# seqan/lambda

Measured on AMD Instinct MI355X. Metric: GCUPS (gapped extension, full-rectangle parity mode; pass-1 cells per second of whole step) searchp BLOSUM62, higher is better.
Workload: dtype f16x2 (exact small integers) + int32

## Files before the change

lambda_amd/csrc/lx_ckpt.hip:

```cpp
#include <hip/hip_runtime.h>

#include <algorithm>
#include <cstdio>
#include <cstdlib>

#include "lx_aids.h"
#include "lx_dp_common.h"

namespace lx
{

#ifndef LX_CKPT_EVERY
#define LX_CKPT_EVERY 16
#endif
constexpr int kCkptEvery = LX_CKPT_EVERY;
#ifndef LX_CKPT_UNROLL
#define LX_CKPT_UNROLL 4
#endif
#define LX_CKPT_PRAGMA(x) _Pragma(#x)
#define LX_CKPT_UNROLL_N(n) LX_CKPT_PRAGMA(unroll n)
#define LX_CKPT_UNROLL_PRAGMA LX_CKPT_UNROLL_N(LX_CKPT_UNROLL)
#ifndef LX_BT_TILE_AT
#define LX_BT_TILE_AT 40
#endif
#ifndef LX_BT_WAVES
#define LX_BT_WAVES 2
#endif
#ifndef LX_BT_HOPS
#define LX_BT_HOPS 2
#endif
#ifndef LX_BT_REFILL_AT
#define LX_BT_REFILL_AT 24
#endif
#ifndef LX_BT_POOL
#define LX_BT_POOL 32
#endif
#ifndef LX_CKPT_FWD_WAVES
#define LX_CKPT_FWD_WAVES 4
#endif
#ifdef LX_BT_COUNT
__device__ unsigned long long lx_bt_counts[5];
#endif

template <int G>
__host__ __device__ constexpr uint32_t bnd_quad_index(uint32_t quad, uint32_t g)
{
    return quad * G + g;
}
#ifndef LX_CKPT_ROWCK_LANE_MAJOR
#define LX_CKPT_ROWCK_LANE_MAJOR 1
#endif
template <int G, int kCkDw>
__host__ __device__ constexpr uint32_t rowck_quad_index(uint32_t m, uint32_t g, uint32_t x)
{
    return LX_CKPT_ROWCK_LANE_MAJOR ? (m * G + g) * (kCkDw / 4) + x : (m * (kCkDw / 4) + x) * G + g;
}
template <int G, int C>
struct CkptLayout
{
    static constexpr int kCkDw = (C + 3) / 4 * 4;
    __host__ __device__ static constexpr uint64_t bnd_dwords(uint32_t steps_cap) { return (uint64_t)steps_cap * G; }
    __host__ __device__ static constexpr uint64_t slot_dwords(uint32_t steps_cap)
    {
        return bnd_dwords(steps_cap) + (uint64_t)(steps_cap / kCkptEvery) * G * kCkDw;
    }
};

__device__ __forceinline__ uint32_t pack16(int lo, int hi)
{
    return ((uint32_t)lo & 0xffffu) | ((uint32_t)hi << 16);
}

template <int G, int C, bool KNOWN, bool MULTI>
__global__ __launch_bounds__(64, (KNOWN ? LX_CKPT_FWD_WAVES : 3)) void ckpt_forward_kernel(TraceParams p)
{
    using Geo = ScoreGeo<G, C>;
    using Lay = CkptLayout<G, C>;
    extern __shared__ uint32_t lds[];

    int const  lane     = threadIdx.x;
    int const  grp      = lane / G;
    int const  g        = lane % G;
    bool const is_first = (g == 0);
    bool const is_last  = (g == G - 1);

    uint64_t const e     = (uint64_t)blockIdx.x * Geo::kGroups + grp;
    uint64_t       limit = p.n;
    if (p.count_ptr)
    {
        uint64_t const total = *p.count_ptr;
        limit = total > p.chunk_start ? min(p.n, total - p.chunk_start) : 0;
        if ((uint64_t)blockIdx.x * Geo::kGroups >= limit)
            return;
    }
    bool active = e < limit;
    if (active && p.src && p.src[e] == 0xffffffffu)
        active = false;
    bool in_list = e < limit;
    if constexpr (!KNOWN)
    {
        if (p.fixup)
        {
            bool const mine = in_list && p.score_out[e] == -1;
            if (__ballot(mine) == 0)
                return;
            active  = active && mine;
            in_list = mine;
        }
    }

    ScoringDev const * __restrict__ sc = p.sc;
    int const      ge    = sc->ge;
    int const      g2    = sc->g2;
    int const      nrows = p.nrows;
    uint32_t const padt  = (uint32_t)(nrows - 1);

    int             lq = 0, ls = 0;
    uint8_t const * q = p.q_res;
    uint8_t const * s = p.s_res;
    uint64_t        q_off = 0;
    if (e < limit)
    {
        Extension const x = p.ext[e];
        lq    = (int)x.q_len;
// ... 289 lines not shown
            grow   = take ? orow : grow;
            gtie   = take ? ot : gtie;
        }
        bool const take = gbest > run_best;
        run_best  = take ? gbest : run_best;
        run_strip = take ? (MULTI ? panel * G : 0) + gstrip : run_strip;
        run_row   = take ? grow : run_row;
        run_tie   = take ? gtie : run_tie;
    }
    if constexpr (MULTI)
    {
        if (npanels > 1)
        {
            __builtin_amdgcn_fence(__ATOMIC_RELEASE, "workgroup");
            __builtin_amdgcn_s_waitcnt(0);
            __builtin_amdgcn_fence(__ATOMIC_ACQUIRE, "workgroup");
        }
    }
    __builtin_amdgcn_wave_barrier();
    }

    if constexpr (KNOWN)
    {
#pragma unroll
        for (int off = 1; off < G; off <<= 1)
        {
            int const  oc = __shfl_xor(kcol, off), orow = __shfl_xor(krow, off);
            bool const take = oc < kcol;
            kcol = take ? oc : kcol;
            krow = take ? orow : krow;
        }
        if (in_list && is_first)
        {
            EndCell ec{};
            if (bad || (tgt > 0 && kcol == 0x7fffffff))
                ec.score = -1;
            else if (tgt > 0)
            {
                ec.score = tgt;
                ec.q_end = kcol + 1;
                ec.s_end = krow + 1;
            }
            p.ends[e] = ec;
        }
    }
    else
    {
        int const gbest = run_best, gstrip = run_strip, grow = run_row, gtie = run_tie;
        if (in_list && is_first)
        {
            EndCell ec{};
            if (bad)
                ec.score = -1;
            else if (active && gbest > 0)
            {
                ec.score = gbest;
                ec.q_end = -(gstrip + 1);
                ec.s_end = grow + 1;
                ec.flags = (gtie ? kEndAmbiguous : 0) | (int32_t)(ovf_tag << kEndOverflowShift);
            }
            p.ends[e] = ec;
            if (p.score_out)
                p.score_out[e] = bad ? -1 : (active ? gbest : 0);
        }
    }
}

template <int G, int C>
__global__ __launch_bounds__(64, LX_BT_WAVES) void ckpt_backtrace_kernel(TraceParams p)
{
    using Lay               = CkptLayout<G, C>;
    using L16               = Ckpt16Layout<G, C>;
    constexpr int kNibDw    = (C + 7) / 8;
    constexpr int kFar      = -(1 << 28);
    static_assert(kCkptEvery == 16, "the diagonal shortcut reads at most 16 residues per sequence");
    __shared__ int8_t   smat4[kAlph * kAlph];
    __shared__ int8_t   smat1n[kAlph * kAlph];
    __shared__ uint32_t tiles[kCkptEvery * kNibDw * 64];
    constexpr int kRecQ  = 10;
    constexpr int kLdsWg = 20 * 1024 - (int)sizeof(uint32_t) * kCkptEvery * kNibDw * 64 - 2 * kAlph * kAlph;
    constexpr int kPool  = LX_BT_POOL < kLdsWg / (16 * kRecQ) ? LX_BT_POOL : kLdsWg / (16 * kRecQ);
    static_assert(kPool >= 0 && kPool <= 64, "pool masks are 64 bits wide");
    __shared__ uint4 pool[kRecQ][kPool > 0 ? kPool : 1];
    for (int x = threadIdx.x; x < kAlph * kAlph; x += blockDim.x)
    {
        int const v = p.sc->mat[x];
        smat4[x]    = (int8_t)((v < -32 || v > 31) ? -125 : 4 * v + 3);
        smat1n[x]   = (int8_t)(x == kAlph * kAlph - 1 ? 0 : min(-v, 127));
    }
    __syncthreads();
    uint32_t const lane  = threadIdx.x;
    uint64_t       limit = p.n;
    if (p.count_ptr)
    {
        uint64_t const total = *p.count_ptr;
        limit = total > p.chunk_start ? min(p.n, total - p.chunk_start) : 0;
    }
    int const ge = p.sc->ge, g2 = p.sc->g2;
    int const ge4 = 4 * p.sc->ge, go4 = 4 * p.sc->go;
    uint64_t panel_dw = Lay::slot_dwords(p.steps_cap), panel16_dw = L16::slot_dwords(p.steps_cap), bnd_dw = Lay::bnd_dwords(p.steps_cap);

    bool             have = false, blocked = false, done = false, need_col = false, scan = false, c16 = false;
    uint64_t         po = 0;
    uint64_t         pos = 0;
    EndCell          ec{};
    uint32_t const * slot = nullptr;
    uint32_t         oct_mul = G, ck_mul = G * (L16::kCkDw / 4);
    uint64_t         ck16_off = 0;
    uint8_t const *  q = nullptr, * s = nullptr;
    uint8_t *        ops_al = nullptr;
    uint32_t         cap = 0, a0 = 0, apos = 0, acc = 0, n = 0;
    int              lq = 0, ls = 0;
    int              i = 0, j = 0, end_i = 0, end_j = 0;
    int              res_col = C, res_row = 0x7fffffff;
    int              nar_cw = C, nar_j0 = 0x7fffffff, nar_st0 = 0x7fffffff;
    auto locate = [&](int aj, int & st, int & j0, int & cw)
    {
        if (aj >= nar_j0)
        {
            int const jl = aj - nar_j0;
            int const gl = nar_cw == (3 * C + 3) / 4 ? jl / ((3 * C + 3) / 4) : nar_cw == (C + 1) / 2 ? jl / ((C + 1) / 2) : jl / ((C + 3) / 4);
            st = nar_st0 + gl;
            j0 = nar_j0 + gl * nar_cw;
            cw = nar_cw;
        }
        else
        {
            st = aj / C;
            j0 = st * C;
            cw = C;
        }
    };
    int              mode = 0;
    int              left = 0;
    int32_t          nm = 0, nx = 0, np = 0, go = 0, gx = 0;
    bool const       rle_mode = p.rle != nullptr;
    uint32_t         run_op = 3, run_len = 0, ncodes = 0;

    auto dec = [](uint32_t bits16) -> int { return (int)(int16_t)bits16; };
    auto expand = [](uint32_t code16) -> uint32_t
    {
        uint32_t const H = code16 & 0x7ffu;
        return H | ((H - (code16 >> 11)) << 16);
    };
    auto bnd_of = [&](uint32_t pn) { return reinterpret_cast<uint4 const *>(slot + (uint64_t)pn * (c16 ? panel16_dw : panel_dw)); };
    auto rowck_of = [&](uint32_t pn)
    {
        return reinterpret_cast<uint4 const *>(slot + (c16 ? (uint64_t)pn * panel16_dw + ck16_off
                                                           : (uint64_t)pn * panel_dw + bnd_dw));
    };
    auto oct16_index = [&](uint32_t o, uint32_t g_) -> uint32_t { return o * oct_mul + g_; };
    auto ck16_index  = [&](uint32_t m_, uint32_t g_, uint32_t x_) -> uint32_t { return m_ * ck_mul + g_ * (L16::kCkDw / 4) + x_; };
    auto rowck_word = [&](uint32_t m, uint32_t st, uint32_t c) -> uint32_t
    {
        if (c16)
            return expand(reinterpret_cast<uint16_t const *>(rowck_of(st / G) + ck16_index(m, st % G, c / 8))[c % 8]);
        return reinterpret_cast<uint32_t const *>(rowck_of(st / G) + rowck_quad_index<G, Lay::kCkDw>(m, st % G, c / 4))[c % 4];
    };
    auto bnd_word_of = [&](uint32_t st, uint32_t k) -> uint32_t
    {
        if (c16)
            return expand(reinterpret_cast<uint16_t const *>(bnd_of(st / G) + oct16_index(k / 8, st % G))[k & 7]);
        return reinterpret_cast<uint32_t const *>(bnd_of(st / G) + bnd_quad_index<G>(k / 4, st % G))[k & 3];
    };
    auto put_byte = [&](uint32_t byte)
    {
        acc |= byte << (8 * (apos & 3));
        if ((apos & 3) == 0)
        {
            if (apos + 3 <= a0 + cap - 1)
                *reinterpret_cast<uint32_t *>(ops_al + apos) = acc;
            else
                for (uint32_t b = 0; b < 4 && apos + b <= a0 + cap - 1; ++b)
                    ops_al[apos + b] = (uint8_t)(acc >> (8 * b));
            acc = 0;
        }
        --apos;
    };
    auto emit = [&](uint32_t op)
    {
        if (rle_mode)
        {
            uint32_t const oc = op == (uint32_t)'M' ? 0u : (op == (uint32_t)'D' ? 1u : 2u);
            if (oc != run_op || run_len == 64)
            {
                if (run_op != 3)
                {
                    put_byte((run_op << 6) | (run_len - 1));
                    ++ncodes;
                }
                run_op  = oc;
                run_len = 0;
            }
            ++run_len;
        }
        else
            put_byte(op);
        ++n;
    };

    auto begin_extension = [&](uint64_t e)
    {
        uint64_t oi = e;
        if (p.src)
        {
            uint32_t const sidx = p.src[e];
            if (sidx == 0xffffffffu)
                return;
            oi = sidx;
        }
        pos                = e;
        po                 = p.out_by_pos ? e : oi;
        uint64_t const  se = p.slot_by_src ? oi : e;
        ec                 = p.ends[se];
        Extension const x  = p.ext[e];
        if (ec.score <= 0)
        {
            Hsp out{};
            out.score     = ec.score < 0 ? -1 : 0;
            p.out_hsp[po] = out;
            return;
        }
        c16                = (ec.flags & kEndCompact) != 0;
        uint32_t const ovf = (uint32_t)ec.flags >> kEndOverflowShift;
        slot               = ovf ? p.ovf + (uint64_t)(ovf - 1) * p.ovf_stride : p.trace + se * p.slot_stride;
        uint32_t steps_e   = p.steps_cap;
        if (p.wf_tab && !ovf)
        {
            WfSlots const  t      = p.wf_tab[se / 16];
            uint64_t const stride = (uint64_t)t.panels_cap * (c16 ? L16::slot_dwords(t.steps_cap) : Lay::slot_dwords(t.steps_cap));
            slot                  = ((p.split_n != 0 && se >= p.split_n) ? p.trace2 : p.trace) + t.off_dw + (se % 16) * stride;
            steps_e               = t.steps_cap;
        }
        panel_dw           = Lay::slot_dwords(steps_e);
        panel16_dw         = L16::slot_dwords(steps_e);
        bnd_dw             = Lay::bnd_dwords(steps_e);
        oct_mul            = G;
        ck_mul             = G * (L16::kCkDw / 4);
        ck16_off           = L16::bnd_dwords(steps_e);
        if (!ovf && (ec.flags & kEndWaveSlots))
        {
            constexpr uint32_t kW = 128 / G;
            uint64_t const     w  = se % kW;
            slot     = p.trace + (se - w) * p.slot_stride + w * (G * 4);
            oct_mul  = kW * G;
            ck_mul   = kW * G * (L16::kCkDw / 4);
// ... 87 lines not shown
            out.s_begin            = i + 1;
            out.s_end              = end_i + 1;
            out.n_ops              = (int32_t)n;
            out.num_matches        = nm;
            out.num_mismatches     = nx;
            out.num_positives      = np;
            out.num_gap_opens      = go;
            out.num_gap_extensions = gx;
            out.ops_shift          = rle_mode ? (int32_t)(uint32_t)at : (int32_t)(cap - n);
        }
        p.out_hsp[po] = out;
        if (rle_mode && p.rle_len)
            p.rle_len[pos] = ec.score > 0 ? ncodes : 0u;
        have          = false;
    };

    auto park = [&](uint32_t e)
    {
        uint32_t const flags = (blocked ? 1u : 0u) | (done ? 2u : 0u) | (need_col ? 4u : 0u) | (scan ? 8u : 0u) | (c16 ? 16u : 0u) |
                               ((uint32_t)mode << 5) | (run_op << 7) | (run_len << 9) | (a0 << 16) | ((uint32_t)nar_cw << 18) |
                               ((uint32_t)res_col << 24);
        uint64_t const sp = reinterpret_cast<uintptr_t>(slot), qp = reinterpret_cast<uintptr_t>(q), spp = reinterpret_cast<uintptr_t>(s),
                       op = reinterpret_cast<uintptr_t>(ops_al);
        pool[0][e] = make_uint4(flags, (uint32_t)pos, (uint32_t)po, (uint32_t)ec.score);
        pool[1][e] = make_uint4((uint32_t)sp, (uint32_t)(sp >> 32), oct_mul, ck_mul);
        pool[2][e] = make_uint4((uint32_t)ck16_off, (uint32_t)panel_dw, (uint32_t)panel16_dw, (uint32_t)bnd_dw);
        pool[3][e] = make_uint4((uint32_t)qp, (uint32_t)(qp >> 32), (uint32_t)spp, (uint32_t)(spp >> 32));
        pool[4][e] = make_uint4((uint32_t)op, (uint32_t)(op >> 32), cap, apos);
        pool[5][e] = make_uint4(acc, n, (uint32_t)lq, (uint32_t)ls);
        pool[6][e] = make_uint4((uint32_t)i, (uint32_t)j, (uint32_t)end_i, (uint32_t)end_j);
        pool[7][e] = make_uint4((uint32_t)res_row, (uint32_t)nar_j0, (uint32_t)nar_st0, (uint32_t)left);
        pool[8][e] = make_uint4((uint32_t)nm, (uint32_t)nx, (uint32_t)np, (uint32_t)go);
        pool[9][e] = make_uint4((uint32_t)gx, ncodes, 0u, 0u);
    };
    auto unpark = [&](uint4 const (&r)[kRecQ])
    {
        uint32_t const flags = r[0].x;
        blocked  = (flags & 1u) != 0;
        done     = (flags & 2u) != 0;
        need_col = (flags & 4u) != 0;
        scan     = (flags & 8u) != 0;
        c16      = (flags & 16u) != 0;
        mode     = (int)((flags >> 5) & 3u);
        run_op   = (flags >> 7) & 3u;
        run_len  = (flags >> 9) & 127u;
        a0       = (flags >> 16) & 3u;
        nar_cw   = (int)((flags >> 18) & 63u);
        res_col  = (int)((flags >> 24) & 63u);
        pos      = r[0].y;
        po       = r[0].z;
        ec.score = (int32_t)r[0].w;
        slot     = reinterpret_cast<uint32_t const *>(((uint64_t)r[1].y << 32) | r[1].x);
        oct_mul  = r[1].z;
        ck_mul   = r[1].w;
        ck16_off   = r[2].x;
        panel_dw   = r[2].y;
        panel16_dw = r[2].z;
        bnd_dw     = r[2].w;
        q      = reinterpret_cast<uint8_t const *>(((uint64_t)r[3].y << 32) | r[3].x);
        s      = reinterpret_cast<uint8_t const *>(((uint64_t)r[3].w << 32) | r[3].z);
        ops_al = reinterpret_cast<uint8_t *>(((uint64_t)r[4].y << 32) | r[4].x);
        cap    = r[4].z;
        apos   = r[4].w;
        acc    = r[5].x;
        n      = r[5].y;
        lq     = (int)r[5].z;
        ls     = (int)r[5].w;
        i      = (int)r[6].x;
        j      = (int)r[6].y;
        end_i  = (int)r[6].z;
        end_j  = (int)r[6].w;
        res_row = (int)r[7].x;
        nar_j0  = (int)r[7].y;
        nar_st0 = (int)r[7].z;
        left    = (int)r[7].w;
        nm      = (int32_t)r[8].x;
        nx      = (int32_t)r[8].y;
        np      = (int32_t)r[8].z;
        go      = (int32_t)r[8].w;
        gx      = (int32_t)r[9].x;
        ncodes  = r[9].y;
        have    = true;
    };
    auto nth_bit = [](uint64_t m, uint32_t r) -> uint32_t
    {
        uint32_t at = 0;
#pragma unroll
        for (int w = 32; w >= 1; w >>= 1)
        {
            uint32_t const lo = (uint32_t)__popcll(m & ((1ull << w) - 1ull));
            if (r >= lo)
            {
                r -= lo;
                m >>= w;
                at += (uint32_t)w;
            }
        }
        return at;
    };
    auto low_bits = [&](uint64_t m, uint32_t r) -> uint64_t
    {
        return r >= (uint32_t)__popcll(m) ? m : (m & ((1ull << nth_bit(m, r)) - 1ull));
    };


    auto load_diagonal = [&](int ci, int cj, int k, uint32_t (&qw)[4], uint32_t (&sw)[4])
    {
#pragma unroll
        for (int d = 0; d < 4; ++d)
        {
            qw[d] = *reinterpret_cast<unaligned_u32 const *>(q + (cj - k + 1) + 4 * d);
            sw[d] = *reinterpret_cast<unaligned_u32 const *>(s + (ci - k + 1) + 4 * d);
        }
    };
    auto take_diagonal = [&](int k, int Hb, bool verify, uint32_t (&qw)[4], uint32_t (&sw)[4]) -> bool
    {
#pragma unroll
        for (int d = 0; d < 4; ++d)
        {
            int const      nb  = k - 4 * d;
            uint32_t const pad = nb >= 4 ? 0u : (nb <= 0 ? 0x1f1f1f1fu : (0x1f1f1f1fu << (8 * nb)));
            qw[d]              = (qw[d] & 0x1f1f1f1fu) | pad;
            sw[d]              = (sw[d] & 0x1f1f1f1fu) | pad;
        }
        int      P = 0, cnt = 0;
        uint32_t posbits = 0;
        int32_t  tmb = 0;
        bool const bs = p.bs_match_rule != 0;
#pragma unroll
        for (int u = kCkptEvery - 1; u >= 0; --u)
        {
            int const      d   = u >> 2, b = u & 3;
            uint32_t const idx = (((qw[d] >> (8 * b)) & 0x1fu) << 5) | ((sw[d] >> (8 * b)) & 0x1fu);
            int const      nv  = (int)smat1n[idx];
            bool const     take = P < left;
            int const      nve = take ? nv : 0;
            cnt += take ? 1 : 0;
            P -= nve;
            posbits = __builtin_amdgcn_alignbit(posbits, (uint32_t)nve, 31);
            if (bs)
                tmb += (take && nv == (int)smat1n[(idx >> 5) * (kAlph + 1)]) ? 1 : 0;
        }
        int const beyond = left > 0 ? kCkptEvery - k : 0;
        cnt -= beyond;
        tmb -= bs ? beyond : 0;
        int const  L       = left - P;
        bool const stopped = cnt < k;
        if (!(stopped ? (L == 0) : (!verify || L == Hb)))
            return false;
        int32_t tm = tmb;
        if (!bs)
        {
            int const lo = k - cnt;
#pragma unroll
            for (int d = 0; d < 4; ++d)
            {
                uint32_t const x   = qw[d] ^ sw[d];
                uint32_t const nz  = (x + 0x7f7f7f7fu) & 0x80808080u;
                int const      b0  = max(lo - 4 * d, 0), b1 = min(k - 4 * d, 4);
                uint32_t const msk = b1 > b0 ? ((b1 >= 4 ? 0xffffffffu : ((1u << (8 * b1)) - 1u)) & ~((1u << (8 * b0)) - 1u)) : 0u;
                tm += __popc(~nz & 0x80808080u & msk);
            }
        }
        left = L;
        nm += tm;
        nx += cnt - tm;
        np += __popc(posbits);
        if (rle_mode)
        {
            int left_m = cnt;
            while (left_m > 0)
            {
                if (run_op != 0 || run_len == 64)
                {
                    if (run_op != 3)
                    {
                        put_byte((run_op << 6) | (run_len - 1));
                        ++ncodes;
                    }
                    run_op  = 0;
                    run_len = 0;
                }
                int const take = min(left_m, 64 - (int)run_len);
                run_len += (uint32_t)take;
                left_m -= take;
            }
        }
        else if (cnt > 0)
        {
            uint32_t const hi = apos, lo = apos + 1 - (uint32_t)cnt, Dtop = hi & ~3u, Dlow = lo & ~3u;
#pragma unroll
            for (int sl = 0; sl < 5; ++sl)
            {
                uint32_t const D = Dtop - 4u * sl;
                if (Dtop >= 4u * sl && D >= Dlow)
                {
                    uint32_t const b0  = lo > D ? lo - D : 0, b1 = sl == 0 ? hi - D : 3u;
                    uint32_t const msk = (b1 >= 3 ? 0xffffffffu : ((1u << (8 * (b1 + 1))) - 1u)) & ~((1u << (8 * b0)) - 1u);
                    uint32_t const val = (sl == 0 ? acc : 0u) | (0x4d4d4d4du & msk);
                    if (lo <= D)
                    {
                        if (sl != 0 || D + 3 <= a0 + cap - 1)
                            *reinterpret_cast<uint32_t *>(ops_al + D) = val;
                        else
                            for (uint32_t bb = 0; bb < 4 && D + bb <= a0 + cap - 1; ++bb)
                                ops_al[D + bb] = (uint8_t)(val >> (8 * bb));
                        acc = 0;
                    }
                    else
                        acc = val;
                }
            }
            apos -= (uint32_t)cnt;
        }
        n += (uint32_t)cnt;
        i -= cnt;
        j -= cnt;
        done = stopped;
        return true;
    };

    bool queue_empty = false;
    int const tile_at = p.bt_tile_at > 0 ? p.bt_tile_at : LX_BT_TILE_AT, refill_at = p.bt_refill_at > 0 ? p.bt_refill_at : LX_BT_REFILL_AT;
#ifdef LX_BT_COUNT
    uint32_t cnt_sc = 0, cnt_sc_lanes = 0, cnt_tile = 0, cnt_tile_lanes = 0;
#endif
    uint64_t pool_used = 0, pool_tile = 0;
    uint64_t const lanes_below = (1ull << lane) - 1ull;
    for (;;)
    {
        bool fin       = have && (done || i < 0 || j < 0 || n >= cap);
        bool can       = have && !fin && !blocked && !need_col && mode == 0;
        bool tile_need = have && !fin && !can;
        int  n_can = __popcll(__ballot(can)), n_tile = __popcll(__ballot(tile_need));
        int const n_idle = 64 - n_can - n_tile;
        int  p_tile = __popcll(pool_tile), p_can = __popcll(pool_used) - p_tile;
        bool run_tile = n_can + p_can == 0 || n_tile + p_tile >= tile_at;
        if (n_idle > 0 && (run_tile || n_idle >= refill_at || n_can == 0))
        {
            if (fin)
                close_ops();
            uint64_t at = 0;
            if (rle_mode)
            {
                uint32_t const mine = fin ? ncodes : 0u;
                uint32_t       incl = mine;
#pragma unroll
                for (int off = 1; off < 64; off <<= 1)
                {
                    uint32_t const up = (uint32_t)__shfl_up((int)incl, off);
                    if ((int)lane >= off)
                        incl += up;
                }
                uint32_t const     total = (uint32_t)__shfl((int)incl, 63);
                unsigned long long base  = 0;
                if (lane == 63 && total != 0)
                    base = atomicAdd(p.rle_top, (unsigned long long)total);
                base = ((unsigned long long)(uint32_t)__shfl((int)(base >> 32), 63) << 32) | (uint32_t)__shfl((int)(uint32_t)base, 63);
                at   = base + incl - mine;
            }
            if (fin)
                finish_extension(at);
            if (!queue_empty)
            {
                if constexpr (kPool > 0)
                {
                    bool const     out = have && !(run_tile ? tile_need : can);
                    uint64_t const mo  = __ballot(out);
                    uint64_t const fr  = ~pool_used & (kPool == 64 ? ~0ull : ((1ull << kPool) - 1ull));
                    uint32_t const npk = min((uint32_t)__popcll(mo), (uint32_t)__popcll(fr));
                    if (npk > 0)
                    {
                        uint32_t const rank = (uint32_t)__popcll(mo & lanes_below);
                        if (out && rank < npk)
                        {
                            park(nth_bit(fr, rank));
                            have = false;
                        }
                        uint64_t const got = low_bits(fr, npk);
                        pool_used |= got;
                        pool_tile |= run_tile ? 0ull : got;
                    }
                }
                uint64_t const want = __ballot(!have);
                if (want != 0)
                {
                    uint32_t  base   = 0;
                    int const leader = __ffsll((unsigned long long)want) - 1;
                    if ((int)lane == leader)
                        base = atomicAdd(p.work_counter, (uint32_t)__popcll(want));
                    base = (uint32_t)__shfl((int)base, leader);
                    if ((uint64_t)base + (uint32_t)__popcll(want) >= limit)
                        queue_empty = true;
                    if (!have)
                    {
                        uint64_t const e = (uint64_t)base + (uint32_t)__popcll(want & ((1ull << lane) - 1ull));
                        if (e < limit)
                            begin_extension(e);
                    }
                }
            }
            fin       = have && (done || i < 0 || j < 0 || n >= cap);
            can       = have && !fin && !blocked && !need_col && mode == 0;
            tile_need = have && !fin && !can;
            n_can     = __popcll(__ballot(can));
            n_tile    = __popcll(__ballot(tile_need));
            if (n_can == 0 && n_tile == 0 && pool_used == 0)
            {
                if (__ballot(have) == 0 && queue_empty)
                {
#ifdef LX_BT_COUNT
                    if (lane == 0)
                    {
                        atomicAdd(&lx_bt_counts[0], (unsigned long long)cnt_sc);
                        atomicAdd(&lx_bt_counts[1], (unsigned long long)cnt_sc_lanes);
                        atomicAdd(&lx_bt_counts[2], (unsigned long long)cnt_tile);
                        atomicAdd(&lx_bt_counts[3], (unsigned long long)cnt_tile_lanes);
                        atomicAdd(&lx_bt_counts[4], 1ull);
                    }
#endif
                    break;
                }
                if (__ballot(have) == 0)
                    continue;
            }
            p_tile   = __popcll(pool_tile);
            p_can    = __popcll(pool_used) - p_tile;
            run_tile = n_can + p_can == 0 || n_tile + p_tile >= tile_at;
        }
        if constexpr (kPool > 0)
        {
            uint64_t const px = run_tile ? pool_tile : (pool_used & ~pool_tile);
            if (px != 0)
            {
                bool const     empty = !have, other = have && !fin && !(run_tile ? tile_need : can);
                uint64_t const me = __ballot(empty), mo = __ballot(other);
                uint32_t const ne = (uint32_t)__popcll(me);
                uint32_t const ns = min((uint32_t)__popcll(px), ne + (uint32_t)__popcll(mo));
                if (ns > 0)
                {
                    uint32_t const rank = empty ? (uint32_t)__popcll(me & lanes_below) : (other ? ne + (uint32_t)__popcll(mo & lanes_below) : 64u);
                    if (rank < ns)
                    {
                        uint32_t const e = nth_bit(px, rank);
                        uint4          r[kRecQ];
#pragma unroll
                        for (int f = 0; f < kRecQ; ++f)
                            r[f] = pool[f][e];
                        if (other)
                            park(e);
                        unpark(r);
                    }
                    uint64_t const taken = low_bits(px, ns), freed = low_bits(px, min(ne, ns));
                    pool_used &= ~freed;
                    pool_tile = (pool_tile & ~freed) ^ (taken & ~freed);
                    fin       = have && (done || i < 0 || j < 0 || n >= cap);
                    can       = have && !fin && !blocked && !need_col && mode == 0;
                    tile_need = have && !fin && !can;
                    n_can     = __popcll(__ballot(can));
                    n_tile    = __popcll(__ballot(tile_need));
                }
            }
        }
#ifdef LX_BT_COUNT
        cnt_sc += run_tile ? 0u : 1u;
        cnt_sc_lanes += run_tile ? 0u : (uint32_t)n_can;
        cnt_tile += run_tile ? 1u : 0u;
        cnt_tile_lanes += run_tile ? (uint32_t)n_tile : 0u;
#endif

        if (!run_tile)
        {
            if (can)
            {
                int      hk[LX_BT_HOPS];
                uint32_t hw[LX_BT_HOPS], hqw[LX_BT_HOPS][4], hsw[LX_BT_HOPS][4];
                int      ci = i, cj = j;
#pragma unroll
                for (int h = 0; h < LX_BT_HOPS; ++h)
                {
                    bool const on = ci >= 0 && cj >= 0;
                    int const ai = max(ci, 0), aj = max(cj, 0);
                    int st, j0, cw;
                    locate(aj, st, j0, cw);
                    int const c  = aj - j0;
                    int const gl = st % G;
                    int const m  = (ai + gl) / kCkptEvery;
                    int const r_base = m * kCkptEvery - gl;
                    int const kt = ai - r_base + 1, kl = c + 1;
                    int const k  = min(min(kt, kl), ai + 1);
                    int const bi = ai - k, bj = aj - k;
                    hk[h] = on ? k : 0;
                    hw[h] = 0;
                    if (on && bi >= 0 && bj >= 0)
                        hw[h] = (kl <= kt) ? bnd_word_of((uint32_t)(st - 1), (uint32_t)(bi + (st - 1) % G))
                                           : rowck_word((uint32_t)(m - 1), (uint32_t)st, (uint32_t)(bj - j0));
                    load_diagonal(ai, aj, k, hqw[h], hsw[h]);
                    ci -= k;
                    cj -= k;
                }
#pragma unroll
                for (int h = 0; h < LX_BT_HOPS; ++h)
                    if (hk[h] > 0 && !blocked && !done)
                        if (!take_diagonal(hk[h], dec(hw[h] & 0xffffu), true, hqw[h], hsw[h]))
                            blocked = true;
            }
            continue;
        }

        if (tile_need)
        {
        int st, j0, cw;
        locate(j, st, j0, cw);
        int const pn = st / G, gl = st % G;
        int const m  = (i + gl) / kCkptEvery;
        int const k_base = m * kCkptEvery;
        int const r_base = k_base - gl;
        uint4 const * const rowck = rowck_of((uint32_t)pn);

        int Hp[C], F[C];
        if (m == 0)
        {
#pragma unroll
            for (int c = 0; c < C; ++c)
            {
                Hp[c] = 0;
                F[c]  = 2;
            }
        }
        else
        {
            uint32_t      w[Lay::kCkDw];
            if (c16)
            {
#pragma unroll
                for (int xq = 0; xq < L16::kCkDw / 4; ++xq)
                {
                    uint4 const    v    = rowck[ck16_index((uint32_t)(m - 1), (uint32_t)gl, (uint32_t)xq)];
                    uint32_t const d[4] = {v.x, v.y, v.z, v.w};
#pragma unroll
                    for (int b = 0; b < 4; ++b)
                    {
                        int const c = 2 * (4 * xq + b);
                        if (c < Lay::kCkDw)
                            w[c] = expand(d[b] & 0xffffu);
                        if (c + 1 < Lay::kCkDw)
                            w[c + 1] = expand(d[b] >> 16);
                    }
                }
            }
            else
            {
#pragma unroll
                for (int xq = 0; xq < Lay::kCkDw / 4; ++xq)
                {
                    uint4 const v = rowck[rowck_quad_index<G, Lay::kCkDw>((uint32_t)(m - 1), (uint32_t)gl, (uint32_t)xq)];
                    w[4 * xq] = v.x; w[4 * xq + 1] = v.y; w[4 * xq + 2] = v.z; w[4 * xq + 3] = v.w;
                }
            }
#pragma unroll
            for (int c = 0; c < C; ++c)
            {
                Hp[c] = 4 * dec(w[c] & 0xffffu);
                F[c]  = (4 * dec(w[c] >> 16)) | 2;
            }
        }
        uint32_t qoff2[(C + 1) / 2];
        uint32_t qd[(C + 3) / 4];
        {
#pragma unroll
            for (int d = 0; d < (C + 3) / 4; ++d)
                qd[d] = *reinterpret_cast<unaligned_u32 const *>(q + j0 + 4 * d);
#pragma unroll
            for (int c = 0; c < C; ++c)
            {
                uint32_t const r = (c < cw && j0 + c < lq) ? ((qd[c >> 2] >> (8 * (c & 3))) & (kAlph - 1)) : (uint32_t)(kAlph - 1);
                qoff2[c >> 1]    = (c & 1) ? (qoff2[c >> 1] | ((r * kAlph) << 16)) : r * kAlph;
            }
        }
        bool const has_left = st > 0;
        int const  gL       = gl > 0 ? gl - 1 : G - 1;
        int const  qshift   = (gl == 0 && has_left) ? G / 4 : 0;
        uint4 const * const bndL = bnd_of((uint32_t)(gl > 0 ? pn : max(pn - 1, 0)));
        auto load_bq = [&](int qd) -> uint4
        {
            if (!has_left || qd + qshift < 0)
                return make_uint4(0, 0, 0, 0);
            if (c16)
            {
                int const   qs = qd + qshift;
                uint2 const v  = reinterpret_cast<uint2 const *>(bndL + oct16_index((uint32_t)qs / 2, (uint32_t)gL))[qs & 1];
                return make_uint4(expand(v.x & 0xffffu), expand(v.x >> 16), expand(v.y & 0xffffu), expand(v.y >> 16));
            }
            return bndL[bnd_quad_index<G>((uint32_t)(qd + qshift), (uint32_t)gL)];
        };
        int const qd0   = k_base / 4;
        uint4     qprev = load_bq(qd0 - 1), qcur = load_bq(qd0);

        uint32_t snext = *reinterpret_cast<unaligned_u32 const *>(s + max(r_base, 0));
#pragma unroll 1
        for (int t = 0; t < kCkptEvery / 4; ++t)
        {
            if (__ballot(r_base + 4 * t <= i) == 0)
                break;
            uint4 const qnext = load_bq(qd0 + t + 1);
            int const      row0 = r_base + 4 * t;
            int const      lb   = max(row0, 0);
            uint32_t const sdw  = snext;
            snext               = *reinterpret_cast<unaligned_u32 const *>(s + max(row0 + 4, 0));
            uint32_t const lw[4] = {qprev.w, qcur.x, qcur.y, qcur.z};
            uint32_t const dw[4] = {qprev.z, qprev.w, qcur.x, qcur.y};
#pragma unroll
            for (int u = 0; u < 4; ++u)
            {
                int const      row = row0 + u;
                uint32_t const tl  = row >= 0 ? (sdw >> (8 * (row - lb))) & (kAlph - 1) : (uint32_t)(kAlph - 1);
                int            E   = (has_left && row >= 0) ? ((4 * dec(lw[u] >> 16)) | 1) : (kFar | 1);
                int            Hd  = (has_left && row > 0) ? 4 * dec(dw[u] & 0xffffu) : 0;
                uint32_t       w[kNibDw];
#pragma unroll
                for (int xw = 0; xw < kNibDw; ++xw)
                    w[xw] = 0;
                int sub4[C];
#pragma unroll
                for (int c = 0; c < C; ++c)
                    sub4[c] = (int)smat4[((qoff2[c >> 1] >> (16 * (c & 1))) & 0xffffu) + tl];
#pragma unroll
                for (int c = 0; c < C; ++c)
                {
                    int const tt  = Hd + sub4[c];
                    Hd            = Hp[c];
                    int const m   = max3i(tt, E, F[c]);
                    int const H4  = m & ~3;
                    int const A   = H4 + go4;
                    int const Fr  = max3i(F[c] + ge4, A, 0);
                    int const Er  = max(E + ge4, A);
                    F[c]          = Fr | 2;
                    E             = Er | 1;
                    Hp[c]         = H4;
                    uint32_t wc   = w[c >> 3];
                    wc            = __builtin_amdgcn_alignbit((uint32_t)m, wc, 2);
                    wc            = __builtin_amdgcn_alignbit((uint32_t)(Fr | Er), wc, 2);
                    w[c >> 3]     = wc;
                }
                int const kk = 4 * t + u;
                w[kNibDw - 1] |= tl;
#pragma unroll
                for (int xw = 0; xw < kNibDw; ++xw)
                    tiles[(kk * kNibDw + xw) * 64 + lane] = w[xw];
                if (need_col && row <= i && row >= 0 && row < ls)
                {
                    int const tgt4 = 4 * ec.score;
                    int       kmax = 0;
#pragma unroll
                    for (int c = 0; c < C; ++c)
                        kmax = max(kmax, ((Hp[c] - tgt4) << 5) + (C - c));
                    int const  cmin  = C - kmax;
                    bool const lower = kmax > 0 && cmin < res_col;
                    res_col          = lower ? cmin : res_col;
                    res_row          = lower ? row : res_row;
                }
            }
            qprev = qcur;
            qcur  = qnext;
        }

        bool walk_ok = true;
        if (scan && r_base + kCkptEvery < ls)
        {
            i       = min(r_base + 2 * kCkptEvery - 1, ls - 1);
            walk_ok = false;
        }
        else if (need_col)
        {
            need_col = false;
            scan     = false;
            walk_ok  = false;
            if (res_col >= C)
            {
                done     = true;
                left     = -1;
                ec.score = -1;
            }
            else
            {
                i     = res_row;
                j     = j0 + res_col;
                end_i = i;
                end_j = j;
            }
        }
        static_assert(32 - 4 * (C - 8 * (kNibDw - 1)) >= 5, "the last nibble word needs 5 spare bits for the subject letter");
        bool passed = false;
        if (walk_ok && mode == 0 && i >= 0 && j >= j0 && i >= r_base)
        {
            int const kk = i - r_base, c = j - j0;
            int const kmax = min(min(kk, c), i) + 1;
            uint32_t  nd = 0;
#pragma unroll
            for (int t = 0; t < kCkptEvery; ++t)
            {
                int const      rr   = max(kk - t, 0), cc = max(c - t, 0);
                int const      xw   = cc >> 3;
                uint32_t const word = tiles[(rr * kNibDw + xw) * 64 + lane];
                int const      sh   = (xw == kNibDw - 1 ? 32 - 4 * (C - 8 * (kNibDw - 1)) : 0) + 4 * (cc & 7);
                nd |= (((word >> sh) & 3u) != 3u) ? (1u << t) : 0u;
            }
            nd |= ~0u << kmax;
            int const d = __ffs((int)nd) - 1;
            if (d > 0)
            {
                uint32_t qw[4], sw[4];
                load_diagonal(i, j, d, qw, sw);
                (void)take_diagonal(d, 0, false, qw, sw);
            }
        }
        while (walk_ok && !done && i >= 0 && j >= j0 && i >= r_base && n < cap && !(passed && mode == 0))
        {
            int const      kk   = i - r_base, c = j - j0;
            int const      xw   = c >> 3;
            int const      cnt  = (xw == kNibDw - 1) ? (C - 8 * xw) : 8;
            uint32_t const word = tiles[(kk * kNibDw + xw) * 64 + lane];
            uint32_t const last = tiles[(kk * kNibDw + (kNibDw - 1)) * 64 + lane];
            uint32_t const nib  = (word >> (32 - 4 * cnt + 4 * (c & 7))) & 15u;
            bool const     in_v = mode == 1, in_h = mode == 2;
            bool const     cont = (in_v && (nib & 8u)) || (in_h && (nib & 4u));
            bool const     leave = (in_v || in_h) && !cont;
            go += leave ? 1 : 0;
            left -= leave ? g2 : 0;
            if (!cont && left <= 0)
            {
                done = true;
                break;
            }
            uint32_t const code = nib & 3u;
            bool const     diag = !cont && code == 3, vert = cont ? in_v : code == 2;
            uint32_t qsel = qd[0];
#pragma unroll
            for (int d = 1; d < (C + 3) / 4; ++d)
                qsel = ((c >> 2) == d) ? qd[d] : qsel;
            uint32_t const c0 = (qsel >> (8 * (c & 3))) & (kAlph - 1), c1 = last & (kAlph - 1);
            int const      sm = (int)smat4[c0 * kAlph + c1];
            int const      v  = (sm - 3) >> 2;
            bool const     isMatch = p.bs_match_rule ? (sm == (int)smat4[c0 * kAlph + c0]) : (c0 == c1);
            nm += (diag && isMatch) ? 1 : 0;
            nx += (diag && !isMatch) ? 1 : 0;
            np += (diag && v > 0) ? 1 : 0;
            gx += cont ? 1 : 0;
            left -= diag ? v : ge;
            mode = diag ? 0 : (vert ? 1 : 2);
            passed = passed || !diag;
            emit(diag ? (uint32_t)'M' : (vert ? (uint32_t)'D' : (uint32_t)'I'));
            i -= (diag || vert) ? 1 : 0;
            j -= (diag || !vert) ? 1 : 0;
        }
        blocked = false;
        }
    }
}


uint64_t ckpt_slot_dwords(int cfg, uint32_t steps_cap)
{
    return cfg == 2   ? CkptLayout<16, 13>::slot_dwords(steps_cap)
           : cfg == 3 ? CkptLayout<8, 13>::slot_dwords(steps_cap)
           : cfg == 4 ? CkptLayout<8, 25>::slot_dwords(steps_cap)
           : cfg == 5 ? CkptLayout<8, 11>::slot_dwords(steps_cap)
                      : CkptLayout<8, 19>::slot_dwords(steps_cap);
}

uint64_t ckpt16_slot_dwords(int cfg, uint32_t steps_cap)
{
    return cfg == 2   ? Ckpt16Layout<16, 13>::slot_dwords(steps_cap)
           : cfg == 3 ? Ckpt16Layout<8, 13>::slot_dwords(steps_cap)
           : cfg == 4 ? Ckpt16Layout<8, 25>::slot_dwords(steps_cap)
           : cfg == 5 ? Ckpt16Layout<8, 11>::slot_dwords(steps_cap)
                      : Ckpt16Layout<8, 19>::slot_dwords(steps_cap);
}

template <int G, int C>
static hipError_t launch_ckpt_forward_cfg(TraceParams const & p, hipStream_t stream)
{
    using Geo = ScoreGeo<G, C>;
    uint64_t const blocks = (p.n + Geo::kGroups - 1) / Geo::kGroups;
    if (blocks > 0x7fffffffull || (!p.score_in && !p.score_out) || p.steps_cap % kCkptEvery != 0)
        return hipErrorInvalidValue;
    int const    share = p.shared_profile > 1 ? std::min(p.shared_profile, Geo::kGroups) : 1;
    int const    slots = (Geo::kGroups + share - 1) / share;
    size_t const lds   = ((size_t)slots * (size_t)p.nrows * Geo::kRowDw + 64 * 4) * sizeof(uint32_t);
    bool const multi = p.panels_cap > 1;
    if (lds > 64 * 1024)
    {
        hipError_t const ea = multi ? hipFuncSetAttribute(reinterpret_cast<void const *>(&ckpt_forward_kernel<G, C, false, true>),
                                                          hipFuncAttributeMaxDynamicSharedMemorySize, (int)lds)
                                    : hipFuncSetAttribute(reinterpret_cast<void const *>(&ckpt_forward_kernel<G, C, false, false>),
                                                          hipFuncAttributeMaxDynamicSharedMemorySize, (int)lds);
        if (ea != hipSuccess || p.score_in)
            return ea != hipSuccess ? ea : hipErrorInvalidValue;
    }
    if (p.score_in && multi)
        hipLaunchKernelGGL((ckpt_forward_kernel<G, C, true, true>), dim3((unsigned)blocks), dim3(64), lds, stream, p);
    else if (p.score_in)
        hipLaunchKernelGGL((ckpt_forward_kernel<G, C, true, false>), dim3((unsigned)blocks), dim3(64), lds, stream, p);
    else if (multi)
        hipLaunchKernelGGL((ckpt_forward_kernel<G, C, false, true>), dim3((unsigned)blocks), dim3(64), lds, stream, p);
    else
        hipLaunchKernelGGL((ckpt_forward_kernel<G, C, false, false>), dim3((unsigned)blocks), dim3(64), lds, stream, p);
    return hipGetLastError();
}

hipError_t launch_ckpt_forward(TraceParams const & p, hipStream_t stream)
{
    if (p.n == 0)
        return hipSuccess;
    return p.cfg == 2   ? launch_ckpt_forward_cfg<16, 13>(p, stream)
           : p.cfg == 3 ? launch_ckpt_forward_cfg<8, 13>(p, stream)
           : p.cfg == 4 ? launch_ckpt_forward_cfg<8, 25>(p, stream)
           : p.cfg == 5 ? launch_ckpt_forward_cfg<8, 11>(p, stream)
                        : launch_ckpt_forward_cfg<8, 19>(p, stream);
}

static int backtrace_resident_waves()
{
    static int const v = []()
    {
        int dev = 0, cus = 256;
        if (hipGetDevice(&dev) == hipSuccess)
            (void)hipDeviceGetAttribute(&cus, hipDeviceAttributeMultiprocessorCount, dev);
        int const per_cu = 4 * LX_BT_WAVES;
        return std::max(1, cus) * per_cu;
    }();
    return v;
}

hipError_t launch_ckpt_backtrace(TraceParams const & p_in, hipStream_t stream)
{
    if (p_in.n == 0)
        return hipSuccess;
    if (!p_in.work_counter)
        return hipErrorInvalidValue;
    TraceParams p = p_in;
    {
        p.bt_tile_at   = dev_aids().bt_tile_at;
        p.bt_refill_at = dev_aids().bt_refill_at;
    }
    uint64_t const b2 = std::min<uint64_t>((p.n + 63) / 64, (uint64_t)backtrace_resident_waves());
    hipError_t e = hipMemsetAsync(p.work_counter, 0, sizeof(uint32_t), stream);
    if (e != hipSuccess)
        return e;
    if (p.cfg == 2)
        hipLaunchKernelGGL((ckpt_backtrace_kernel<16, 13>), dim3((unsigned)b2), dim3(64), 0, stream, p);
    else if (p.cfg == 3)
        hipLaunchKernelGGL((ckpt_backtrace_kernel<8, 13>), dim3((unsigned)b2), dim3(64), 0, stream, p);
    else if (p.cfg == 4)
        hipLaunchKernelGGL((ckpt_backtrace_kernel<8, 25>), dim3((unsigned)b2), dim3(64), 0, stream, p);
    else if (p.cfg == 5)
        hipLaunchKernelGGL((ckpt_backtrace_kernel<8, 11>), dim3((unsigned)b2), dim3(64), 0, stream, p);
    else
        hipLaunchKernelGGL((ckpt_backtrace_kernel<8, 19>), dim3((unsigned)b2), dim3(64), 0, stream, p);
#ifdef LX_BT_COUNT
    {
        unsigned long long c[5] = {};
        e = hipGetLastError();
        if (e == hipSuccess)
            e = hipStreamSynchronize(stream);
        if (e == hipSuccess)
            e = hipMemcpyFromSymbol(c, HIP_SYMBOL(lx_bt_counts), sizeof(c));
        unsigned long long const z[5] = {};
        if (e == hipSuccess)
            e = hipMemcpyToSymbol(HIP_SYMBOL(lx_bt_counts), z, sizeof(z));
        if (e != hipSuccess)
            return e;
        fprintf(stderr, "LX_BT_COUNT cfg %d n %llu waves %llu: shortcut passes %llu, lanes/pass %.2f; tile phases %llu, lanes/phase %.2f\n",
                p.cfg, (unsigned long long)p.n, c[4], c[0], c[0] ? (double)c[1] / (double)c[0] : 0.0, c[2],
                c[2] ? (double)c[3] / (double)c[2] : 0.0);
    }
#endif
    return hipGetLastError();
}

}
```

Measured before the change: 5669.

## Profile backtrace sections and streamline bit-rank, word loads and run writes

Adds optional per-section cycle counters to the checkpoint backtrace kernel, active only when LX_BT_COUNT is defined. Several hot helpers change at the same time. nth_bit and low_bits become wave-wide permute and ballot operations instead of a serial binary search. The hop word loads become aligned dword loads with deferred decode. The diagonal match mask is simplified, and the run of 'M' opcodes is written with a closed-form path instead of a five-slot loop. The permute-based nth_bit now executes on every lane unconditionally, which adds cross-lane traffic on paths that only some lanes needed.

```diff
diff --git a/lambda_amd/csrc/lx_ckpt.hip b/lambda_amd/csrc/lx_ckpt.hip
--- a/lambda_amd/csrc/lx_ckpt.hip
+++ b/lambda_amd/csrc/lx_ckpt.hip
@@ -40,6 +40,32 @@
 #endif
 #ifdef LX_BT_COUNT
 __device__ unsigned long long lx_bt_counts[5];
+enum BtSection
+{
+    kBtCtrl = 0,
+    kBtRetire,
+    kBtExchange,
+    kBtHopSetup,
+    kBtHopBody,
+    kBtTileSetup,
+    kBtTileDp,
+    kBtTileScan,
+    kBtTileWalk,
+    kBtSections
+};
+__device__ unsigned long long lx_bt_cycles[kBtSections + 5];
+#define LX_BT_MARK(sec)                                                    \
+    do                                                                     \
+    {                                                                      \
+        unsigned long long const bt_now_ = (unsigned long long)clock64();  \
+        if (lane == (uint32_t)(__ffsll(__ballot(true)) - 1))               \
+        {                                                                  \
+            bt_lds[sec] += bt_now_ - bt_lds[kBtSections];                  \
+            bt_lds[kBtSections] = bt_now_;                                 \
+        }                                                                  \
+    } while (0)
+#else
+#define LX_BT_MARK(sec) do {} while (0)
 #endif
 
 template <int G>
@@ -495,6 +521,9 @@
     constexpr int kPool  = LX_BT_POOL < kLdsWg / (16 * kRecQ) ? LX_BT_POOL : kLdsWg / (16 * kRecQ);
     static_assert(kPool >= 0 && kPool <= 64, "pool masks are 64 bits wide");
     __shared__ uint4 pool[kRecQ][kPool > 0 ? kPool : 1];
+#ifdef LX_BT_COUNT
+    unsigned long long const bt_entry = (unsigned long long)clock64();
+#endif
     for (int x = threadIdx.x; x < kAlph * kAlph; x += blockDim.x)
     {
         int const v = p.sc->mat[x];
@@ -564,17 +593,25 @@
     };
     auto oct16_index = [&](uint32_t o, uint32_t g_) -> uint32_t { return o * oct_mul + g_; };
     auto ck16_index  = [&](uint32_t m_, uint32_t g_, uint32_t x_) -> uint32_t { return m_ * ck_mul + g_ * (L16::kCkDw / 4) + x_; };
-    auto rowck_word = [&](uint32_t m, uint32_t st, uint32_t c) -> uint32_t
+    auto rowck_word_addr = [&](uint32_t m, uint32_t st, uint32_t c) -> uint8_t const *
     {
         if (c16)
-            return expand(reinterpret_cast<uint16_t const *>(rowck_of(st / G) + ck16_index(m, st % G, c / 8))[c % 8]);
-        return reinterpret_cast<uint32_t const *>(rowck_of(st / G) + rowck_quad_index<G, Lay::kCkDw>(m, st % G, c / 4))[c % 4];
-    };
-    auto bnd_word_of = [&](uint32_t st, uint32_t k) -> uint32_t
+            return reinterpret_cast<uint8_t const *>(reinterpret_cast<uint16_t const *>(rowck_of(st / G) + ck16_index(m, st % G, c / 8)) + c % 8);
+        return reinterpret_cast<uint8_t const *>(reinterpret_cast<uint32_t const *>(rowck_of(st / G) + rowck_quad_index<G, Lay::kCkDw>(m, st % G, c / 4)) + c % 4);
+    };
+    auto bnd_word_addr = [&](uint32_t st, uint32_t k) -> uint8_t const *
     {
         if (c16)
-            return expand(reinterpret_cast<uint16_t const *>(bnd_of(st / G) + oct16_index(k / 8, st % G))[k & 7]);
-        return reinterpret_cast<uint32_t const *>(bnd_of(st / G) + bnd_quad_index<G>(k / 4, st % G))[k & 3];
+            return reinterpret_cast<uint8_t const *>(reinterpret_cast<uint16_t const *>(bnd_of(st / G) + oct16_index(k / 8, st % G)) + (k & 7));
+        return reinterpret_cast<uint8_t const *>(reinterpret_cast<uint32_t const *>(bnd_of(st / G) + bnd_quad_index<G>(k / 4, st % G)) + (k & 3));
+    };
+    auto dword_around = [](uint8_t const * a) -> uint32_t
+    {
+        return *reinterpret_cast<uint32_t const *>(reinterpret_cast<uintptr_t>(a) & ~(uintptr_t)3);
+    };
+    auto h_of_dword = [&](uint32_t dw, uint32_t upper_half) -> int
+    {
+        return c16 ? (int)((dw >> (upper_half ? 16 : 0)) & 0x7ffu) : (int)(int16_t)(dw & 0xffffu);
     };
     auto put_byte = [&](uint32_t byte)
     {
@@ -828,25 +865,16 @@
         ncodes  = r[9].y;
         have    = true;
     };
-    auto nth_bit = [](uint64_t m, uint32_t r) -> uint32_t
-    {
-        uint32_t at = 0;
-#pragma unroll
-        for (int w = 32; w >= 1; w >>= 1)
-        {
-            uint32_t const lo = (uint32_t)__popcll(m & ((1ull << w) - 1ull));
-            if (r >= lo)
-            {
-                r -= lo;
-                m >>= w;
-                at += (uint32_t)w;
-            }
-        }
-        return at;
+    auto nth_bit = [&](uint64_t m, uint32_t r) -> uint32_t
+    {
+        uint32_t const below = (uint32_t)__popcll(m & ((1ull << lane) - 1ull));
+        uint32_t const dest  = ((m >> lane) & 1ull) ? below : (uint32_t)__popcll(m) + (lane - below);
+        int const      nth   = __builtin_amdgcn_ds_permute((int)(dest << 2), (int)lane);
+        return (uint32_t)__builtin_amdgcn_ds_bpermute((int)((r & 63u) << 2), nth);
     };
     auto low_bits = [&](uint64_t m, uint32_t r) -> uint64_t
     {
-        return r >= (uint32_t)__popcll(m) ? m : (m & ((1ull << nth_bit(m, r)) - 1ull));
+        return __ballot(((m >> lane) & 1ull) != 0 && (uint32_t)__popcll(m & ((1ull << lane) - 1ull)) < r);
     };
 
 
@@ -903,10 +931,11 @@
             {
                 uint32_t const x   = qw[d] ^ sw[d];
                 uint32_t const nz  = (x + 0x7f7f7f7fu) & 0x80808080u;
-                int const      b0  = max(lo - 4 * d, 0), b1 = min(k - 4 * d, 4);
-                uint32_t const msk = b1 > b0 ? ((b1 >= 4 ? 0xffffffffu : ((1u << (8 * b1)) - 1u)) & ~((1u << (8 * b0)) - 1u)) : 0u;
+                int const      b0  = min(max(lo - 4 * d, 0), 4);
+                uint32_t const msk = b0 >= 4 ? 0u : (0xffffffffu << (8 * b0));
                 tm += __popc(~nz & 0x80808080u & msk);
             }
+            tm -= kCkptEvery - k;
         }
         left = L;
         nm += tm;
@@ -934,28 +963,23 @@
         }
         else if (cnt > 0)
         {
-            uint32_t const hi = apos, lo = apos + 1 - (uint32_t)cnt, Dtop = hi & ~3u, Dlow = lo & ~3u;
-#pragma unroll
-            for (int sl = 0; sl < 5; ++sl)
-            {
-                uint32_t const D = Dtop - 4u * sl;
-                if (Dtop >= 4u * sl && D >= Dlow)
-                {
-                    uint32_t const b0  = lo > D ? lo - D : 0, b1 = sl == 0 ? hi - D : 3u;
-                    uint32_t const msk = (b1 >= 3 ? 0xffffffffu : ((1u << (8 * (b1 + 1))) - 1u)) & ~((1u << (8 * b0)) - 1u);
-                    uint32_t const val = (sl == 0 ? acc : 0u) | (0x4d4d4d4du & msk);
-                    if (lo <= D)
-                    {
-                        if (sl != 0 || D + 3 <= a0 + cap - 1)
-                            *reinterpret_cast<uint32_t *>(ops_al + D) = val;
-                        else
-                            for (uint32_t bb = 0; bb < 4 && D + bb <= a0 + cap - 1; ++bb)
-                                ops_al[D + bb] = (uint8_t)(val >> (8 * bb));
-                        acc = 0;
-                    }
-                    else
-                        acc = val;
-                }
+            uint32_t const top = apos & 3u, D = apos & ~3u;
+            if ((uint32_t)cnt <= top)
+                acc |= (0x4d4d4d4du >> (8 * (4 - cnt))) << (8 * (top + 1 - (uint32_t)cnt));
+            else
+            {
+                uint32_t const val = acc | (0x4d4d4d4du >> (8 * (3 - top)));
+                if (D + 3 <= a0 + cap - 1)
+                    *reinterpret_cast<uint32_t *>(ops_al + D) = val;
+                else
+                    for (uint32_t bb = 0; bb < 4 && D + bb <= a0 + cap - 1; ++bb)
+                        ops_al[D + bb] = (uint8_t)(val >> (8 * bb));
+                uint32_t const rem = (uint32_t)cnt - (top + 1), whole = rem >> 2, tail = rem & 3u;
+#pragma unroll
+                for (uint32_t w = 1; w <= 3; ++w)
+                    if (w <= whole)
+                        *reinterpret_cast<uint32_t *>(ops_al + D - 4u * w) = 0x4d4d4d4du;
+                acc = tail ? 0x4d4d4d4du << (8 * (4 - tail)) : 0u;
             }
             apos -= (uint32_t)cnt;
         }
@@ -970,6 +994,14 @@
     int const tile_at = p.bt_tile_at > 0 ? p.bt_tile_at : LX_BT_TILE_AT, refill_at = p.bt_refill_at > 0 ? p.bt_refill_at : LX_BT_REFILL_AT;
 #ifdef LX_BT_COUNT
     uint32_t cnt_sc = 0, cnt_sc_lanes = 0, cnt_tile = 0, cnt_tile_lanes = 0;
+    __shared__ unsigned long long bt_lds[kBtSections + 1];
+    uint32_t walk_iters = 0, walk_lane_iters = 0, walk_max = 0;
+    if (lane == 0)
+    {
+        for (int x = 0; x < kBtSections; ++x)
+            bt_lds[x] = 0;
+        bt_lds[kBtSections] = (unsigned long long)clock64();
+    }
 #endif
     uint64_t pool_used = 0, pool_tile = 0;
     uint64_t const lanes_below = (1ull << lane) - 1ull;
@@ -984,6 +1016,7 @@
         bool run_tile = n_can + p_can == 0 || n_tile + p_tile >= tile_at;
         if (n_idle > 0 && (run_tile || n_idle >= refill_at || n_can == 0))
         {
+            LX_BT_MARK(kBtCtrl);
             if (fin)
                 close_ops();
             uint64_t at = 0;
@@ -1018,9 +1051,10 @@
                     if (npk > 0)
                     {
                         uint32_t const rank = (uint32_t)__popcll(mo & lanes_below);
+                        uint32_t const to = nth_bit(fr, rank);
                         if (out && rank < npk)
                         {
-                            park(nth_bit(fr, rank));
+                            park(to);
                             have = false;
                         }
                         uint64_t const got = low_bits(fr, npk);
@@ -1056,6 +1090,7 @@
                 if (__ballot(have) == 0 && queue_empty)
                 {
 #ifdef LX_BT_COUNT
+                    LX_BT_MARK(kBtRetire);
                     if (lane == 0)
                     {
                         atomicAdd(&lx_bt_counts[0], (unsigned long long)cnt_sc);
@@ -1063,20 +1098,32 @@
                         atomicAdd(&lx_bt_counts[2], (unsigned long long)cnt_tile);
                         atomicAdd(&lx_bt_counts[3], (unsigned long long)cnt_tile_lanes);
                         atomicAdd(&lx_bt_counts[4], 1ull);
+                        for (int x = 0; x < kBtSections; ++x)
+                            atomicAdd(&lx_bt_cycles[x], bt_lds[x]);
+                        atomicAdd(&lx_bt_cycles[kBtSections], (unsigned long long)walk_iters);
+                        atomicAdd(&lx_bt_cycles[kBtSections + 1], (unsigned long long)walk_lane_iters);
+                        atomicAdd(&lx_bt_cycles[kBtSections + 2], (unsigned long long)cnt_tile);
+                        atomicMax(&lx_bt_cycles[kBtSections + 3], (unsigned long long)walk_max);
+                        atomicAdd(&lx_bt_cycles[kBtSections + 4], (unsigned long long)clock64() - bt_entry);
                     }
 #endif
                     break;
                 }
                 if (__ballot(have) == 0)
+                {
+                    LX_BT_MARK(kBtRetire);
                     continue;
+                }
             }
             p_tile   = __popcll(pool_tile);
             p_can    = __popcll(pool_used) - p_tile;
             run_tile = n_can + p_can == 0 || n_tile + p_tile >= tile_at;
+            LX_BT_MARK(kBtRetire);
         }
         if constexpr (kPool > 0)
         {
             uint64_t const px = run_tile ? pool_tile : (pool_used & ~pool_tile);
+            LX_BT_MARK(kBtCtrl);
             if (px != 0)
             {
                 bool const     empty = !have, other = have && !fin && !(run_tile ? tile_need : can);
@@ -1086,9 +1133,10 @@
                 if (ns > 0)
                 {
                     uint32_t const rank = empty ? (uint32_t)__popcll(me & lanes_below) : (other ? ne + (uint32_t)__popcll(mo & lanes_below) : 64u);
+                    uint32_t const from = nth_bit(px, rank);
                     if (rank < ns)
                     {
-                        uint32_t const e = nth_bit(px, rank);
+                        uint32_t const e = from;
                         uint4          r[kRecQ];
 #pragma unroll
                         for (int f = 0; f < kRecQ; ++f)
@@ -1107,6 +1155,7 @@
                     n_tile    = __popcll(__ballot(tile_need));
                 }
             }
+            LX_BT_MARK(kBtExchange);
         }
 #ifdef LX_BT_COUNT
         cnt_sc += run_tile ? 0u : 1u;
@@ -1117,10 +1166,12 @@
 
         if (!run_tile)
         {
+            LX_BT_MARK(kBtCtrl);
             if (can)
             {
                 int      hk[LX_BT_HOPS];
                 uint32_t hw[LX_BT_HOPS], hqw[LX_BT_HOPS][4], hsw[LX_BT_HOPS][4];
+                uint32_t hf[LX_BT_HOPS];
                 int      ci = i, cj = j;
 #pragma unroll
                 for (int h = 0; h < LX_BT_HOPS; ++h)
@@ -1137,23 +1188,32 @@
                     int const k  = min(min(kt, kl), ai + 1);
                     int const bi = ai - k, bj = aj - k;
                     hk[h] = on ? k : 0;
-                    hw[h] = 0;
-                    if (on && bi >= 0 && bj >= 0)
-                        hw[h] = (kl <= kt) ? bnd_word_of((uint32_t)(st - 1), (uint32_t)(bi + (st - 1) % G))
-                                           : rowck_word((uint32_t)(m - 1), (uint32_t)st, (uint32_t)(bj - j0));
+                    bool const           inside = on && bi >= 0 && bj >= 0;
+                    uint8_t const *      wa     = reinterpret_cast<uint8_t const *>(slot);
+                    if (inside)
+                        wa = (kl <= kt) ? bnd_word_addr((uint32_t)(st - 1), (uint32_t)(bi + (st - 1) % G))
+                                        : rowck_word_addr((uint32_t)(m - 1), (uint32_t)st, (uint32_t)(bj - j0));
+                    hw[h] = dword_around(wa);
+                    hf[h] = (inside ? 1u : 0u) | ((uint32_t)(reinterpret_cast<uintptr_t>(wa) & 2u));
                     load_diagonal(ai, aj, k, hqw[h], hsw[h]);
                     ci -= k;
                     cj -= k;
                 }
+                LX_BT_MARK(kBtHopSetup);
 #pragma unroll
                 for (int h = 0; h < LX_BT_HOPS; ++h)
                     if (hk[h] > 0 && !blocked && !done)
-                        if (!take_diagonal(hk[h], dec(hw[h] & 0xffffu), true, hqw[h], hsw[h]))
+                        if (!take_diagonal(hk[h], (hf[h] & 1u) ? h_of_dword(hw[h], hf[h] & 2u) : 0, true, hqw[h], hsw[h]))
                             blocked = true;
+                LX_BT_MARK(kBtHopBody);
             }
             continue;
         }
 
+        LX_BT_MARK(kBtCtrl);
+#ifdef LX_BT_COUNT
+        uint32_t my_walk = 0;
+#endif
         if (tile_need)
         {
         int st, j0, cw;
@@ -1244,6 +1304,7 @@
         uint4     qprev = load_bq(qd0 - 1), qcur = load_bq(qd0);
 
         uint32_t snext = *reinterpret_cast<unaligned_u32 const *>(s + max(r_base, 0));
+        LX_BT_MARK(kBtTileSetup);
 #pragma unroll 1
         for (int t = 0; t < kCkptEvery / 4; ++t)
         {
@@ -1310,6 +1371,7 @@
             qprev = qcur;
             qcur  = qnext;
         }
+        LX_BT_MARK(kBtTileDp);
 
         bool walk_ok = true;
         if (scan && r_base + kCkptEvery < ls)
@@ -1361,8 +1423,12 @@
                 (void)take_diagonal(d, 0, false, qw, sw);
             }
         }
+        LX_BT_MARK(kBtTileScan);
         while (walk_ok && !done && i >= 0 && j >= j0 && i >= r_base && n < cap && !(passed && mode == 0))
         {
+#ifdef LX_BT_COUNT
+            ++my_walk;
+#endif
             int const      kk   = i - r_base, c = j - j0;
             int const      xw   = c >> 3;
             int const      cnt  = (xw == kNibDw - 1) ? (C - 8 * xw) : 8;
@@ -1401,7 +1467,22 @@
             j -= (diag || !vert) ? 1 : 0;
         }
         blocked = false;
-        }
+        LX_BT_MARK(kBtTileWalk);
+        }
+#ifdef LX_BT_COUNT
+        {
+            uint32_t wmax = my_walk, wsum = my_walk;
+            for (int off = 32; off >= 1; off >>= 1)
+            {
+                wmax = max(wmax, (uint32_t)__shfl_xor((int)wmax, off));
+                wsum += (uint32_t)__shfl_xor((int)wsum, off);
+            }
+            wmax = (uint32_t)__builtin_amdgcn_readfirstlane((int)wmax);
+            walk_iters += wmax;
+            walk_lane_iters += (uint32_t)__builtin_amdgcn_readfirstlane((int)wsum);
+            walk_max = max(walk_max, wmax);
+        }
+#endif
     }
 }
 
@@ -1520,6 +1601,24 @@
         fprintf(stderr, "LX_BT_COUNT cfg %d n %llu waves %llu: shortcut passes %llu, lanes/pass %.2f; tile phases %llu, lanes/phase %.2f\n",
                 p.cfg, (unsigned long long)p.n, c[4], c[0], c[0] ? (double)c[1] / (double)c[0] : 0.0, c[2],
                 c[2] ? (double)c[3] / (double)c[2] : 0.0);
+        unsigned long long cy[kBtSections + 5] = {};
+        e = hipMemcpyFromSymbol(cy, HIP_SYMBOL(lx_bt_cycles), sizeof(cy));
+        unsigned long long const zc[kBtSections + 5] = {};
+        if (e == hipSuccess)
+            e = hipMemcpyToSymbol(HIP_SYMBOL(lx_bt_cycles), zc, sizeof(zc));
+        if (e != hipSuccess)
+            return e;
+        static char const * const names[kBtSections] = {"control", "retire/refill", "pool exchange", "hop setup", "hop body", "tile setup",
+                                                         "tile DP rows", "tile scan", "tile walk"};
+        double total = 0;
+        for (int x = 0; x < kBtSections; ++x)
+            total += (double)cy[x];
+        fprintf(stderr, "LX_BT_COUNT wave cycles by section (sum %.4g = %.1f %% of the wavefronts' %.4g from entry to exit):", total,
+                cy[kBtSections + 4] ? 100.0 * total / (double)cy[kBtSections + 4] : 0.0, (double)cy[kBtSections + 4]);
+        for (int x = 0; x < kBtSections; ++x)
+            fprintf(stderr, " %s %.4g (%.1f %%);", names[x], (double)cy[x], total > 0 ? 100.0 * (double)cy[x] / total : 0.0);
+        fprintf(stderr, "\nLX_BT_COUNT walk: %llu iterations of the wavefronts (%llu of single lanes) in %llu tile phases, at most %llu in one phase\n",
+                cy[kBtSections], cy[kBtSections + 1], cy[kBtSections + 2], cy[kBtSections + 3]);
     }
 #endif
     return hipGetLastError();
```

Result: faster. 5770 (median of 6 runs) (+1.8%).
